# Zhaohuai-L/Any-Stereo

Hardware: AMD Instinct MI355X
Metric: stereo pairs/sec (coreContinuous_IGEV inference, 32-iter GRU, 960x540) (higher is better)
Workload: dtype f32 (3xf16 split-precision MFMA, fp32 accumulate); 1 GPU; coreContinuous_IGEV inference, 960x540 SceneFlow-shape synthetic pair (padded 960x544), 32 GRU iters, scale 1.0, Q=518400 queries, 1 pair(s) per GPU, random-init weights; pairs_per_gpu=1, parallelism=replicas x1, gru_loop=hipGraph

## Files before the change

any-stereo_amd/csrc/conv.hip:

```cpp
#include <stdlib.h>

#include <type_traits>

#include "common.h"
#include "conv_plan.h"
#include "split.h"

namespace {

using namespace as;

struct ConvParams {
  const float* src[AS_MAX_SRCS];
  int src_c[AS_MAX_SRCS];
  int src_end[AS_MAX_SRCS];
  int n_src;
  const float* wpack;
  const float* bias;
  const float* add;
  int add_ctot, add_coff;
  const float* h;
  const float* z;
  float* out;
  float* out2;
  int out_ctot, out_coff;
  int B, H, W, Cin, Cout, Cout_pad, act;
  int Hi, Wi;
  int tiles_x, tiles_y, n_tiles, chunks;
  int src_bs[AS_MAX_SRCS];
  _Float16* out_bs;
  int out_bs_c8tot, out_bs_coff8;
  int out_bs_ctot;
  int bs_only;
  int all_bs;
  int dual;
  const float* src2;
  int src2_bs;
  const float* wpack2;
  const float* bias2;
  int out_coff2, out_bs_coff8_2;
  const float* h2;
  int act2;
  int dual_sep;
  float* out_b;
  _Float16* out_bs_b;
  const float* tap_w;
  int xcd_map;
  int fast16;
  int ksplit;
  float* ws;
  int stagger;
  int lean_offset;
};

constexpr int kEpiTaps = AS_EPI_RELU_TAPS;

template <int KS> struct ConvCfg;
template <> struct ConvCfg<3> { static constexpr int KC = 8; };
template <> struct ConvCfg<1> { static constexpr int KC = 32; };
static_assert(ConvCfg<3>::KC == conv_kc(3) && ConvCfg<1>::KC == conv_kc(1), "conv_igemm_kernel's K chunk is the planner's");

struct EpiCtx {
  __amdgpu_buffer_rsrc_t r_add, r_out, r_h, r_z, r_bs, r_bsl;
  bool has_add, has_bs, skip_out;
  int act;
  int cvalid;
  int cend;
  unsigned plane4;
};

template <int EPI>
__device__ __forceinline__ EpiCtx make_epi_ctx(const ConvParams& p, int b, int n0, int bn, bool second = false) {
  EpiCtx e;
  const long long plane = (long long)p.H * p.W;
  const int cvalid = min(p.Cout - n0, bn);
  const int recs = cvalid > 0 ? (int)((long long)cvalid * plane * 4) : 0;
  e.plane4 = (unsigned)(plane * 4);
  e.act = second ? p.act2 : p.act;
  const bool sep = second && p.dual_sep;
  e.has_add = p.add != nullptr;
  const float* addp = p.add ? p.add + ((long long)b * p.add_ctot + p.add_coff + n0) * plane : p.out;
  e.r_add = __builtin_amdgcn_make_buffer_rsrc((void*)addp, 0, p.add ? recs : 0, 0x00020000);
  if (EPI == kEpiPartial) {
    const int ks = (int)(blockIdx.x / ((unsigned)p.B * p.tiles_x * p.tiles_y * p.n_tiles));
    float* dst = p.ws + (((long long)ks * p.B + b) * p.Cout_pad + n0) * plane;
    e.r_out = __builtin_amdgcn_make_buffer_rsrc((void*)dst, 0, (int)((long long)bn * plane * 4), 0x00020000);
    e.r_add = __builtin_amdgcn_make_buffer_rsrc((void*)dst, 0, 0, 0x00020000);
    e.has_add = false;
    e.r_h = e.r_out;
    e.r_z = e.r_out;
  } else if (EPI == AS_EPI_LINEAR) {
    float* outp = sep ? p.out_b + ((long long)b * p.Cout + n0) * plane
                      : p.out + ((long long)b * p.out_ctot + (second ? p.out_coff2 : p.out_coff) + n0) * plane;
    e.r_out = __builtin_amdgcn_make_buffer_rsrc((void*)outp, 0, recs, 0x00020000);
    const float* hsel = second ? p.h2 : p.h;
    const float* res = hsel ? hsel + ((long long)b * p.Cout + n0) * plane : outp;
    e.r_h = __builtin_amdgcn_make_buffer_rsrc((void*)res, 0, hsel ? recs : 0, 0x00020000);
    e.r_z = e.r_out;
  } else if (EPI == AS_EPI_GRU_ZR) {
    const int ch = p.Cout >> 1;
    const bool is_r = n0 >= ch;
    const int c0 = is_r ? n0 - ch : n0;
    float* dst = (is_r ? p.out2 : p.out) + ((long long)b * ch + c0) * plane;
    e.r_out = __builtin_amdgcn_make_buffer_rsrc((void*)dst, 0, recs, 0x00020000);
    e.r_h = __builtin_amdgcn_make_buffer_rsrc((void*)(p.h + ((long long)b * ch + c0) * plane), 0, is_r ? recs : 0, 0x00020000);
    e.r_z = e.r_out;
  } else {
    const long long o = ((long long)b * p.Cout + n0) * plane;
    e.r_out = __builtin_amdgcn_make_buffer_rsrc((void*)(p.out + o), 0, recs, 0x00020000);
    e.r_h = __builtin_amdgcn_make_buffer_rsrc((void*)(p.h + o), 0, recs, 0x00020000);
    e.r_z = __builtin_amdgcn_make_buffer_rsrc((void*)(p.z + o), 0, recs, 0x00020000);
  }
  e.has_bs = false;
  e.skip_out = false;
  e.cvalid = cvalid;
  e.cend = cvalid;
  e.r_bs = e.r_out;
  e.r_bsl = e.r_out;
  if (EPI != kEpiPartial && (sep ? p.out_bs_b != nullptr : p.out_bs != nullptr)) {
    int c0 = n0;
    bool on = true;
    if (EPI == AS_EPI_GRU_ZR) { const int ch = p.Cout >> 1; on = n0 >= ch; c0 = n0 - ch; }
    if (on) {
      const int nblk = cvalid > 0 ? (cvalid + 7) / 8 : 0;
      const int coff8 = sep ? 0 : (second ? p.out_bs_coff8_2 : p.out_bs_coff8);
      const int c8tot = sep ? (p.Cout + 7) / 8 : p.out_bs_c8tot;
      _Float16* dst = (sep ? p.out_bs_b : p.out_bs) + (((long long)b * 2 * c8tot + coff8 + (c0 >> 3)) * plane) * 8;
      e.r_bs = __builtin_amdgcn_make_buffer_rsrc((void*)dst, 0, (int)((long long)nblk * plane * 16), 0x00020000);
      e.r_bsl = __builtin_amdgcn_make_buffer_rsrc((void*)(dst + (long long)c8tot * plane * 8), 0, (int)((long long)nblk * plane * 16), 0x00020000);
      e.has_bs = true;
      e.cend = (sep ? p.Cout : p.out_bs_ctot) - (coff8 * 8 + c0);
      e.skip_out = p.bs_only != 0;
    }
  }
  return e;
}

__device__ unsigned g_split_overflow_conv;

struct EpiRegs {
  unsigned off[8];
  float av[8], hv[8], zv[8];
};

template <int EPI>
__device__ __forceinline__ void epi_load(const EpiCtx& e, int col0, int half, unsigned poff, int g, EpiRegs& R) {
  constexpr unsigned kOOB = 0x7FFFFFF0u;
#pragma unroll
  for (int i = 0; i < 8; ++i) {
    const int r = g * 8 + i;
    const int col = col0 + (r & 3) + 8 * (r >> 2) + 4 * half;
    R.off[i] = poff == kOOB ? kOOB : (unsigned)col * e.plane4 + poff;
    R.av[i] = bload(e.r_add, R.off[i]);
    if (EPI == AS_EPI_GRU_ZR || EPI == AS_EPI_LINEAR) R.hv[i] = bload(e.r_h, R.off[i]);
    if (EPI == AS_EPI_GRU_Q) { R.hv[i] = bload(e.r_h, R.off[i]); R.zv[i] = bload(e.r_z, R.off[i]); }
  }
}

// ... 245 lines not shown
#pragma unroll
  for (int t = 0; t < 4; ++t) {
    if (t == wave) continue;
    const int slot = t * 3 + (wave < t ? wave : wave - 1);
    float* dst = lds + slot * 1024 + lane;
#pragma unroll
    for (int r = 0; r < 16; ++r) dst[r * 64] = acc[t >> 1][t & 1][r];
  }
  __syncthreads();
  f32x16 sum;
  {
    const f32x16 own = (wave == 0) ? acc[0][0] : (wave == 1) ? acc[0][1] : (wave == 2) ? acc[1][0] : acc[1][1];
    sum = own;
    const float* srcp = lds + wave * 3 * 1024 + lane;
#pragma unroll
    for (int s = 0; s < 3; ++s)
#pragma unroll
      for (int r = 0; r < 16; ++r) sum[r] += srcp[s * 1024 + r * 64];
  }

  __syncthreads();
  if (tid < kBN) lds[tid] = (p.bias && n0 + tid < p.Cout) ? p.bias[n0 + tid] : 0.f;
  __syncthreads();
  {
    const EpiCtx e = make_epi_ctx<EPI>(p, b, n0, kBN);
    const int m = (wave & 1) * 32 + l31;
    const int gy = y0 + m / TW, gx = x0 + m % TW;
    const unsigned poff = (gy < p.H && gx < p.W) ? (unsigned)(((long long)gy * p.W + gx) * 4) : 0x7FFFFFF0u;
    const bool is_r = (EPI == AS_EPI_GRU_ZR) && n0 >= (p.Cout >> 1);
    epilogue_tile<EPI>(p, e, sum, (wave >> 1) * 32, half, poff, lds, is_r);
  }
}

__global__ void pack_weights_kernel(const float* __restrict__ w, float* __restrict__ wp, int Cin, int Cout,
                                    int Cout_pad, int KS, int KC, long long total) {
  const long long idx = (long long)blockIdx.x * 256 + threadIdx.x;
  if (idx >= total) return;
  const int co = (int)(idx % Cout_pad);
  long long t = idx / Cout_pad;
  const int cl = (int)(t % KC);
  t /= KC;
  const int tap = (int)(t % (KS * KS));
  const int chunk = (int)(t / (KS * KS));
  const int ci = chunk * KC + cl;
  float v = 0.f;
  if (co < Cout && ci < Cin) v = w[((long long)co * Cin + ci) * KS * KS + tap];
  wp[idx] = v;
}


__global__ __launch_bounds__(256) void conv7x7_c1_kernel(const float* __restrict__ x, const float* __restrict__ w,
                                                         const float* __restrict__ bias, float* __restrict__ out,
                                                         int H, int W, int Cout, int out_ctot, int out_coff) {
  __shared__ float patch[22 * 22];
  const int b = blockIdx.z;
  const int x0 = blockIdx.x * 16, y0 = blockIdx.y * 16;
  const long long plane = (long long)H * W;
  const float* xp = x + (long long)b * plane;
  for (int idx = threadIdx.x; idx < 22 * 22; idx += 256) {
    const int py = idx / 22, px = idx - py * 22;
    const int gy = y0 - 3 + py, gx = x0 - 3 + px;
    patch[idx] = (gy >= 0 && gy < H && gx >= 0 && gx < W) ? xp[(long long)gy * W + gx] : 0.f;
  }
  __syncthreads();
  const int ly = threadIdx.x >> 4, lx = threadIdx.x & 15;
  float win[49];
#pragma unroll
  for (int t = 0; t < 49; ++t) win[t] = patch[(ly + t / 7) * 22 + lx + t % 7];
  const int gy = y0 + ly, gx = x0 + lx;
  const bool ok = gy < H && gx < W;
  float* o = out + ((long long)b * out_ctot + out_coff) * plane + (long long)gy * W + gx;
  for (int co = 0; co < Cout; ++co) {
    float acc = 0.f;
#pragma unroll
    for (int t = 0; t < 49; ++t) acc += win[t] * w[co * 49 + t];
    acc += bias ? bias[co] : 0.f;
    if (ok) o[(long long)co * plane] = fmaxf(acc, 0.f);
  }
}

__device__ __forceinline__ void bs8_store(_Float16* __restrict__ out_bs, long long b, int c8tot, int blk, long long plane,
                                          long long pix, const float (&v)[8], float& amax) {
  half8 hi, lo;
  amax = amax8(v, amax);
  split_mode8(v, hi, lo);
  _Float16* rec = out_bs + ((b * 2 * c8tot + blk) * plane + pix) * 8;
  *reinterpret_cast<half8*>(rec) = hi;
  *reinterpret_cast<half8*>(rec + (long long)c8tot * plane * 8) = lo;
}

template <int CO>
__global__ __launch_bounds__(256) void conv7x7_c1_tm_kernel(const float* __restrict__ x, const float* __restrict__ wt,
                                                            const float* __restrict__ bias, float* __restrict__ out,
                                                            int H, int W, int Cout, int CP, int out_ctot, int out_coff,
                                                            float* __restrict__ copy_out, int copy_ctot, int copy_coff, int copy_bs,
                                                            int out_bs) {
  __shared__ float patch[22 * 22];
  as::fp16_saturate_mode();
  float ovf_amax = 0.f;
  const int groups = CP / CO;
  const int b = blockIdx.z / groups;
  const int c0 = (blockIdx.z - b * groups) * CO;
  const int x0 = blockIdx.x * 16, y0 = blockIdx.y * 16;
  const long long plane = (long long)H * W;
  const __amdgpu_buffer_rsrc_t rs = __builtin_amdgcn_make_buffer_rsrc((void*)(x + (long long)b * plane), 0, (int)(plane * 4), 0x00020000);
  for (int idx = threadIdx.x; idx < 22 * 22; idx += 256) {
    const int py = idx / 22, px = idx - py * 22;
    const int gy = y0 - 3 + py, gx = x0 - 3 + px;
    patch[idx] = bload(rs, (gy >= 0 && gy < H && gx >= 0 && gx < W) ? (unsigned)((gy * W + gx) * 4) : 0x7FFFFFF0u);
  }
  __syncthreads();
  const int ly = threadIdx.x >> 4, lx = threadIdx.x & 15;
  float acc[CO];
#pragma unroll
  for (int j = 0; j < CO; ++j) acc[j] = 0.f;
#pragma unroll 1
  for (int ky = 0; ky < 7; ++ky) {
    const float* pr = patch + (ly + ky) * 22 + lx;
    const float* wr = wt + (ky * 7) * CP + c0;
#pragma unroll
    for (int kx = 0; kx < 7; ++kx) {
      const float v = pr[kx];
#pragma unroll
      for (int j = 0; j < CO; ++j) acc[j] = fmaf(v, wr[kx * CP + j], acc[j]);
    }
  }
  const int gy = y0 + ly, gx = x0 + lx;
  if (gy < H && gx < W) {
    if (out_bs) {
      static_assert(CO == 8, "blocked output: one 8-channel block per thread");
      if (c0 < (Cout + 7) / 8 * 8) {
        float v[8];
#pragma unroll
        for (int j = 0; j < CO; ++j) v[j] = (c0 + j < Cout) ? fmaxf(acc[j] + (bias ? bias[c0 + j] : 0.f), 0.f) : 0.f;
        bs8_store(reinterpret_cast<_Float16*>(out), b, (out_ctot + 7) >> 3, (out_coff + c0) >> 3, plane, (long long)gy * W + gx, v, ovf_amax);
      }
    } else {
      float* o = out + ((long long)b * out_ctot + out_coff + c0) * plane + (long long)gy * W + gx;
#pragma unroll
      for (int j = 0; j < CO; ++j)
        if (c0 + j < Cout) o[(long long)j * plane] = fmaxf(acc[j] + (bias ? bias[c0 + j] : 0.f), 0.f);
    }
    if (copy_out && c0 == 0) {
      const float v = patch[(ly + 3) * 22 + lx + 3];
      if (copy_bs) {
        const int c8 = (copy_ctot + 7) >> 3;
        _Float16* rec = reinterpret_cast<_Float16*>(copy_out) + (((long long)b * 2 * c8 + (copy_coff >> 3)) * plane + (long long)gy * W + gx) * 8 + (copy_coff & 7);
        const _Float16 hk = split_hi(v);
        rec[0] = hk;
        rec[(long long)c8 * plane * 8] = split_lo(v, hk);
        ovf_amax = fmaxf(ovf_amax, fabsf(v));
      } else {
        copy_out[((long long)b * copy_ctot + copy_coff) * plane + (long long)gy * W + gx] = v;
      }
    }
  }
  as::note_split_overflow(ovf_amax, &g_split_overflow_conv);
}

__global__ __launch_bounds__(256) void conv3x3_to1_kernel(const float* __restrict__ x, const float* __restrict__ w,
                                                          const float* __restrict__ bias, float* __restrict__ out,
                                                          int Cin, int H, int W) {
  __shared__ float red[4][64];
  const int lx = threadIdx.x & 63, slice = threadIdx.x >> 6;
  const int gx = blockIdx.x * 64 + lx, gy = blockIdx.y, b = blockIdx.z;
  const long long plane = (long long)H * W;
  const int c0 = slice * ((Cin + 3) / 4), c1 = min(Cin, c0 + (Cin + 3) / 4);
  float acc = 0.f;
  if (gx < W) {
    for (int c = c0; c < c1; ++c) {
      const float* xp = x + ((long long)b * Cin + c) * plane;
      const float* wc = w + c * 9;
#pragma unroll
      for (int ky = 0; ky < 3; ++ky) {
        const int yy = gy + ky - 1;
        if (yy < 0 || yy >= H) continue;
#pragma unroll
        for (int kx = 0; kx < 3; ++kx) {
          const int xx = gx + kx - 1;
          const float v = (xx >= 0 && xx < W) ? xp[(long long)yy * W + xx] : 0.f;
          acc += v * wc[ky * 3 + kx];
        }
      }
    }
  }
  red[slice][lx] = acc;
  __syncthreads();
  if (slice == 0 && gx < W)
    out[(long long)b * plane + (long long)gy * W + gx] = ((red[0][lx] + red[1][lx]) + (red[2][lx] + red[3][lx])) + (bias ? bias[0] : 0.f);
}

__global__ __launch_bounds__(256) void tap_shift_sum_kernel(const float* __restrict__ S, const float* __restrict__ bias,
                                                            const float* __restrict__ addend, float* __restrict__ out, int H,
                                                            int W, long long P, int groups) {
  const long long pix = (long long)blockIdx.x * 256 + threadIdx.x;
  if (pix >= P) return;
  const long long plane = (long long)H * W;
  const long long b = pix / plane;
  const int rem = (int)(pix - b * plane);
  const int y = rem / W, x = rem - y * W;
  const float* sp = S + b * groups * 9 * plane;
  float acc = 0.f;
  const __amdgpu_buffer_rsrc_t rs = __builtin_amdgcn_make_buffer_rsrc((void*)sp, 0, (int)((long long)groups * 9 * plane * 4), 0x00020000);
  unsigned toff[9];
#pragma unroll
  for (int t = 0; t < 9; ++t) {
    const int yy = y + t / 3 - 1, xx = x + t % 3 - 1;
    toff[t] = (yy >= 0 && yy < H && xx >= 0 && xx < W) ? (unsigned)(((long long)t * plane + (long long)yy * W + xx) * 4) : 0x7FFFFFF0u;
  }
  const unsigned gstep = (unsigned)(9 * plane * 4);
  for (int g0 = 0; g0 < groups; g0 += 4) {
    float v[4][9];
#pragma unroll
    for (int g = 0; g < 4; ++g)
#pragma unroll
      for (int t = 0; t < 9; ++t)
        v[g][t] = bload(rs, (toff[t] == 0x7FFFFFF0u || g0 + g >= groups) ? 0x7FFFFFF0u : toff[t] + (unsigned)(g0 + g) * gstep);
#pragma unroll
    for (int g = 0; g < 4; ++g)
#pragma unroll
      for (int t = 0; t < 9; ++t) acc += v[g][t];
  }
  const float delta = acc + (bias ? bias[0] : 0.f);
  out[pix] = addend ? addend[pix] + delta : delta;
}

__device__ __forceinline__ float pool2x_at(const float* __restrict__ xp, int yo, int xo, int H, int W) {
  float s = 0.f;
#pragma unroll
  for (int dy = 0; dy < 3; ++dy) {
    const int yy = 2 * yo - 1 + dy;
    if (yy < 0 || yy >= H) continue;
#pragma unroll
    for (int dx = 0; dx < 3; ++dx) {
      const int xx = 2 * xo - 1 + dx;
      if (xx >= 0 && xx < W) s += xp[(long long)yy * W + xx];
    }
  }
  return s / 9.f;
}

__global__ __launch_bounds__(256) void pool2x_kernel(const float* __restrict__ x, float* __restrict__ out, int H, int W,
                                                     int Ho, int Wo, long long total) {
  const long long idx = (long long)blockIdx.x * 256 + threadIdx.x;
  if (idx >= total) return;
  const int xo = (int)(idx % Wo);
  long long t = idx / Wo;
  const int yo = (int)(t % Ho);
  const long long bc = t / Ho;
  out[idx] = pool2x_at(x + bc * H * W, yo, xo, H, W);
}

__global__ __launch_bounds__(256) void pool2x_bs_kernel(const float* __restrict__ x, _Float16* __restrict__ out_bs, int C, int H, int W,
                                                        int Ho, int Wo, long long total) {
  const long long idx = (long long)blockIdx.x * 256 + threadIdx.x;
  as::fp16_saturate_mode();
  float ovf_amax = 0.f;
  if (idx >= total) return;
  const int c8 = (C + 7) >> 3;
  const int xo = (int)(idx % Wo);
  long long t = idx / Wo;
  const int yo = (int)(t % Ho);
  t /= Ho;
  const int blk = (int)(t % c8);
  const long long b = t / c8;
  const long long plane = (long long)H * W;
  const int nch = min(8, C - blk * 8);
  const __amdgpu_buffer_rsrc_t rs = __builtin_amdgcn_make_buffer_rsrc((void*)(x + (b * C + blk * 8) * plane), 0, (int)(nch * plane * 4), 0x00020000);
  unsigned off[9];
#pragma unroll
  for (int k = 0; k < 9; ++k) {
    const int yy = 2 * yo - 1 + k / 3, xx = 2 * xo - 1 + k % 3;
    off[k] = (yy >= 0 && yy < H && xx >= 0 && xx < W) ? (unsigned)(((long long)yy * W + xx) * 4) : 0x7FFFFFF0u;
  }
  const unsigned pl4 = (unsigned)(plane * 4);
  float raw[8][9];
#pragma unroll
  for (int j = 0; j < 8; ++j)
#pragma unroll
    for (int k = 0; k < 9; ++k) raw[j][k] = bload(rs, off[k] == 0x7FFFFFF0u ? off[k] : off[k] + (unsigned)j * pl4);
  float v[8];
#pragma unroll
  for (int j = 0; j < 8; ++j) {
    float sacc = 0.f;
#pragma unroll
    for (int k = 0; k < 9; ++k) sacc += raw[j][k];
    v[j] = sacc / 9.f;
  }
  bs8_store(out_bs, b, c8, blk, (long long)Ho * Wo, (long long)yo * Wo + xo, v, ovf_amax);
  as::note_split_overflow(ovf_amax, &g_split_overflow_conv);
}

__global__ __launch_bounds__(256) void pool2x_bs_even_kernel(const float* __restrict__ x, _Float16* __restrict__ out_bs, int C, int H, int W,
                                                             int Ho, int Wo, long long total) {
  const long long idx0 = (long long)blockIdx.x * 256 + threadIdx.x;
  as::fp16_saturate_mode();
  float ovf_amax = 0.f;
  const bool live = idx0 < total;
  const long long idx = live ? idx0 : total - 1;
  const int c8 = (C + 7) >> 3;
  const int xo = (int)(idx % Wo);
  long long t = idx / Wo;
  const int yo = (int)(t % Ho);
  t /= Ho;
  const int blk = (int)(t % c8);
  const long long b = t / c8;
// ... 935 lines not shown
  static_assert(!LEAN || lds <= 80 * 1024, "conv_split (lean): two blocks per CU");
  static bool configured = false;
  if (!configured && lds > 64 * 1024) {
    (void)hipFuncSetAttribute((const void*)conv_split_kernel<KS, TW, BN, EPI, NSUB, S, FAST, LEAN>, hipFuncAttributeMaxDynamicSharedMemorySize, lds);
    configured = true;
  }
  hipLaunchKernelGGL((conv_split_kernel<KS, TW, BN, EPI, NSUB, S, FAST, LEAN>), dim3((unsigned)pl.grid), dim3(pl.block), pl.lds, s, p);
  return as::check_launch("conv2d(split)");
}

template <int... Vs> struct Among {};
template <class F> bool conv_switch(F f) { f(); return true; }
template <class F, int... Vs, class... Rest>
bool conv_switch(F f, Among<Vs...>, int v, Rest... rest) {
  return ((v == Vs && conv_switch([&](auto... cs) { f(std::integral_constant<int, Vs>{}, cs...); }, rest...)) || ...);
}

int conv_launch(const ConvParams& p, const ConvPlan& pl, hipStream_t s) {
  int rc = 1;
  if (pl.family == kConvIgemm) {
    conv_switch([&](auto ks, auto tw, auto epi) {
      if constexpr (conv_igemm_valid(ks(), tw(), epi())) {
        hipLaunchKernelGGL((conv_igemm_kernel<ks(), tw(), epi()>), dim3((unsigned)pl.grid), dim3(pl.block), 0, s, p);
        rc = as::check_launch("conv2d");
      }
    }, Among<1, 3>{}, pl.KS, Among<8, 16, 32, 64>{}, pl.TW, Among<0, 1, 2>{}, pl.epilogue);
  } else if (pl.family == kConvSplit) {
    conv_switch([&](auto ks, auto tw, auto bn, auto epi, auto nsub, auto st, auto fast, auto lean) {
      if constexpr (conv_split_valid(ks(), tw(), bn(), epi(), nsub(), st(), fast(), lean()))
        rc = launch_conv_split<ks(), tw(), bn(), epi(), nsub(), st(), fast() != 0, lean() != 0>(p, pl, s);
    }, Among<1, 3>{}, pl.KS, Among<16, 32, 128>{}, pl.TW, Among<64, 128>{}, pl.BN, Among<0, 1, 2, 3, 4>{}, pl.epilogue,
       Among<1, 2>{}, pl.NSUB, Among<1, 2>{}, pl.S, Among<0, 1>{}, pl.FAST != 0, Among<0, 1>{}, pl.LEAN != 0);
  }
  return rc <= 0 ? rc : conv_no_kernel(pl);
}

int conv_run(const as_conv_desc& d, const ConvPlan& pl, hipStream_t s) {
  const ConvParams p = conv_fill_params(d, pl);
  const int rc = conv_launch(p, pl, s);
  if (rc != AS_OK || !pl.finish) return rc;
  const dim3 g((unsigned)pl.finish_grid);
  if (pl.finish_epilogue == AS_EPI_LINEAR) hipLaunchKernelGGL(conv_finish_kernel<AS_EPI_LINEAR>, g, dim3(256), 0, s, p);
  else if (pl.finish_epilogue == AS_EPI_GRU_ZR) hipLaunchKernelGGL(conv_finish_kernel<AS_EPI_GRU_ZR>, g, dim3(256), 0, s, p);
  else hipLaunchKernelGGL(conv_finish_kernel<AS_EPI_GRU_Q>, g, dim3(256), 0, s, p);
  return as::check_launch("conv2d(split-K finish)");
}

}

bool as::conv_has_kernel(const as_conv_plan& pl) {
  return pl.family == kConvIgemm ? conv_igemm_valid(pl.KS, pl.TW, pl.epilogue)
                                 : pl.family == kConvSplit && conv_split_valid(pl.KS, pl.TW, pl.BN, pl.epilogue, pl.NSUB, pl.S, pl.FAST != 0, pl.LEAN != 0);
}

extern "C" {

#ifdef AS_CONV_STAMPS
int as_debug_conv_stamps(unsigned long long* out, int n) {
  if (!out || n <= 0 || n > kStampBlocks * kStampSlots) return AS_ERR_BAD_ARG;
  if (hipMemcpyFromSymbol(out, HIP_SYMBOL(as_conv_stamp_buf), sizeof(unsigned long long) * n) != hipSuccess) return AS_ERR_LAUNCH;
  static unsigned long long zeros[kStampBlocks * kStampSlots];
  if (hipMemcpyToSymbol(HIP_SYMBOL(as_conv_stamp_buf), zeros, sizeof(zeros)) != hipSuccess) return AS_ERR_LAUNCH;
  return AS_OK;
}
int as_debug_conv_life(unsigned long long* out, int n) {
  if (!out || n <= 0 || n > kStampBlocks * 8) return AS_ERR_BAD_ARG;
  if (hipMemcpyFromSymbol(out, HIP_SYMBOL(as_conv_life_buf), sizeof(unsigned long long) * n) != hipSuccess) return AS_ERR_LAUNCH;
  return AS_OK;
}
#endif

int64_t as_conv_pack_size(int Cin, int Cout, int KS) {
  if (Cin <= 0 || Cout <= 0 || (KS != 1 && KS != 3)) return -1;
  const int KC = conv_kc(KS);
  const int64_t chunks = (Cin + KC - 1) / KC;
  return chunks * KS * KS * KC * conv_cout_pad(Cout);
}

int as_conv_pack_weights(const float* weight, float* wpack, int Cin, int Cout, int KS, void* stream) {
  AS_REQUIRE(weight && wpack, AS_ERR_BAD_ARG, "conv_pack: null pointer");
  const int64_t total = as_conv_pack_size(Cin, Cout, KS);
  AS_REQUIRE(total > 0, AS_ERR_BAD_ARG, "conv_pack: unsupported Cin=%d Cout=%d KS=%d", Cin, Cout, KS);
  hipLaunchKernelGGL(pack_weights_kernel, dim3((unsigned)as::cdiv64(total, 256)), dim3(256), 0, as::as_stream(stream),
                     weight, wpack, Cin, Cout, conv_cout_pad(Cout), KS, conv_kc(KS), (long long)total);
  return as::check_launch("conv_pack_weights");
}

int64_t as_conv_pack_size_split(int Cin, int Cout, int KS) {
  if (Cin <= 0 || Cout <= 0 || (KS != 1 && KS != 3)) return -1;
  int64_t chunks = (Cin + kSplitKC - 1) / kSplitKC;
  if (KS == 1) chunks = (chunks + 3) / 4 * 4;
  return chunks * KS * KS * 4 * conv_cout_pad(Cout) * 8;
}

int as_conv_pack_weights_split_t(const float* weight, void* wpack, int Cin, int Cout, int KS, void* stream) {
  AS_REQUIRE(weight && wpack, AS_ERR_BAD_ARG, "conv_pack_split_t: null pointer");
  const int64_t total = as_conv_pack_size_split(Cin, Cout, KS);
  AS_REQUIRE(total > 0, AS_ERR_BAD_ARG, "conv_pack_split_t: unsupported Cin=%d Cout=%d KS=%d", Cin, Cout, KS);
  hipLaunchKernelGGL(pack_weights_split_kernel, dim3((unsigned)as::cdiv64(total, 256)), dim3(256), 0, as::as_stream(stream),
                     weight, (_Float16*)wpack, Cin, Cout, conv_cout_pad(Cout), KS * KS, (long long)total, 1);
  return as::check_launch("conv_pack_weights_split_t");
}

int as_conv_pack_weights_split(const float* weight, void* wpack, int Cin, int Cout, int KS, void* stream) {
  AS_REQUIRE(weight && wpack, AS_ERR_BAD_ARG, "conv_pack_split: null pointer");
  const int64_t total = as_conv_pack_size_split(Cin, Cout, KS);
  AS_REQUIRE(total > 0, AS_ERR_BAD_ARG, "conv_pack_split: unsupported Cin=%d Cout=%d KS=%d", Cin, Cout, KS);
  hipLaunchKernelGGL(pack_weights_split_kernel, dim3((unsigned)as::cdiv64(total, 256)), dim3(256), 0, as::as_stream(stream),
                     weight, (_Float16*)wpack, Cin, Cout, conv_cout_pad(Cout), KS * KS, (long long)total, 0);
  return as::check_launch("conv_pack_weights_split");
}

int64_t as_conv_ws_elems(int B, int Cout, int H, int W) {
  if (B <= 0 || Cout <= 0 || H <= 0 || W <= 0) return 0;
  const int cpad = conv_cout_pad(Cout);
  const int bn = (cpad % 128 == 0) ? 128 : 64;
  const long long tiles = (long long)B * as::cdiv64((long long)H * W, 128) * (cpad / bn);
  const int ks = conv_ksplit_cap(tiles, 8);
  return ks > 1 ? (int64_t)ks * B * cpad * H * W : 0;
}

int as_conv2d(const as_conv_desc* d, void* stream) {
  int rc = as::conv_validate(d);
  if (rc != AS_OK) return rc;
  const int fast16 = as::fast16_mode();
  hipStream_t s = as::as_stream(stream);
  ConvPlan pl;
  if ((rc = conv_plan(*d, conv_knobs(), fast16, &pl)) != AS_OK) return rc;
  if (pl.dual != kDualSequential) return conv_run(*d, pl, s);
  as_conv_desc first = *d;
  first.dual = 0;
  const as_conv_desc second = as::conv_dual_second(*d);
  ConvPlan pl2;
  if ((rc = as::conv_validate(&second)) != AS_OK || (rc = conv_plan(second, conv_knobs(), fast16, &pl2)) != AS_OK) return rc;
  if ((rc = conv_run(first, pl, s)) != AS_OK) return rc;
  return conv_run(second, pl2, s);
}

int as_conv7x7_c1_relu(const float* x, const float* weight, const float* bias, float* out, int B, int H, int W,
                       int Cout, int out_ctot, int out_coff, int tap_major, float* copy_out, int copy_ctot, int copy_coff,
                       int copy_bs, int out_bs, void* stream) {
  AS_REQUIRE(x && weight && out, AS_ERR_BAD_ARG, "conv7x7_c1: null pointer");
  AS_REQUIRE((long long)H * W * 4 < 0x7FFFFFF0ll, AS_ERR_BAD_SHAPE, "conv7x7_c1: plane too large");
  AS_REQUIRE(B > 0 && H > 0 && W > 0 && Cout > 0, AS_ERR_BAD_ARG, "conv7x7_c1: non-positive size");
  AS_REQUIRE(out_coff >= 0 && out_coff + Cout <= (out_bs ? (out_ctot + 7) / 8 * 8 : out_ctot), AS_ERR_BAD_SHAPE, "conv7x7_c1: out channel window outside out_ctot");
  AS_REQUIRE(!out_bs || (out_coff % 8 == 0 && (reinterpret_cast<uintptr_t>(out) & 15) == 0), AS_ERR_BAD_ARG, "conv7x7_c1: blocked output window must start at a multiple of 8, 16-B aligned");
  AS_REQUIRE(B <= 65535 && as::cdiv(H, 16) <= 65535, AS_ERR_BAD_SHAPE, "conv7x7_c1: grid too large");
  dim3 grid((unsigned)as::cdiv(W, 16), (unsigned)as::cdiv(H, 16), (unsigned)B);
  if (tap_major) {
    const int CP = (Cout + 63) / 64 * 64;
    AS_REQUIRE((long long)B * (CP / 8) <= 65535, AS_ERR_BAD_SHAPE, "conv7x7_c1: grid too large");
    const dim3 g3(grid.x, grid.y, (unsigned)(B * (CP / 8)));
    AS_REQUIRE(!copy_out || (copy_coff >= 0 && copy_coff < copy_ctot), AS_ERR_BAD_SHAPE, "conv7x7_c1: copy channel outside copy_ctot");
    hipLaunchKernelGGL(conv7x7_c1_tm_kernel<8>, g3, dim3(256), 0, as::as_stream(stream), x, weight, bias, out, H, W, Cout, CP, out_ctot, out_coff,
                       copy_out, copy_ctot, copy_coff, copy_bs, out_bs);
  } else {
    AS_REQUIRE(!out_bs, AS_ERR_BAD_ARG, "conv7x7_c1: a blocked output needs tap_major weights");
    AS_REQUIRE(!copy_out, AS_ERR_BAD_ARG, "conv7x7_c1: the input pass-through needs tap_major weights");
    hipLaunchKernelGGL(conv7x7_c1_kernel, grid, dim3(256), 0, as::as_stream(stream), x, weight, bias, out, H, W, Cout, out_ctot, out_coff);
  }
  return as::check_launch("conv7x7_c1_relu");
}

int as_conv3x3_to1(const float* x, const float* weight, const float* bias, float* out, int B, int Cin, int H, int W, void* stream) {
  AS_REQUIRE(x && weight && out, AS_ERR_BAD_ARG, "conv3x3_to1: null pointer");
  AS_REQUIRE(B > 0 && H > 0 && W > 0 && Cin > 0, AS_ERR_BAD_ARG, "conv3x3_to1: non-positive size");
  AS_REQUIRE(B <= 65535 && H <= 65535, AS_ERR_BAD_SHAPE, "conv3x3_to1: grid too large");
  dim3 grid((unsigned)as::cdiv(W, 64), (unsigned)H, (unsigned)B);
  hipLaunchKernelGGL(conv3x3_to1_kernel, grid, dim3(256), 0, as::as_stream(stream), x, weight, bias, out, Cin, H, W);
  return as::check_launch("conv3x3_to1");
}

int as_tap_shift_sum(const float* S, const float* bias, const float* addend, float* out, int B, int H, int W, int groups, void* stream) {
  AS_REQUIRE(S && out, AS_ERR_BAD_ARG, "tap_shift_sum: null pointer");
  AS_REQUIRE(B > 0 && H > 0 && W > 0 && groups > 0, AS_ERR_BAD_ARG, "tap_shift_sum: non-positive size");
  const long long P = (long long)B * H * W;
  hipLaunchKernelGGL(tap_shift_sum_kernel, dim3((unsigned)as::cdiv64(P, 256)), dim3(256), 0, as::as_stream(stream), S, bias, addend, out, H, W, P, groups);
  return as::check_launch("tap_shift_sum");
}

int as_pool2x(const float* x, float* out, int B, int C, int H, int W, void* stream) {
  AS_REQUIRE(x && out, AS_ERR_BAD_ARG, "pool2x: null pointer");
  AS_REQUIRE(B > 0 && C > 0 && H > 0 && W > 0, AS_ERR_BAD_ARG, "pool2x: non-positive size");
  const int Ho = (H - 1) / 2 + 1, Wo = (W - 1) / 2 + 1;
  const long long total = (long long)B * C * Ho * Wo;
  hipLaunchKernelGGL(pool2x_kernel, dim3((unsigned)as::cdiv64(total, 256)), dim3(256), 0, as::as_stream(stream), x, out, H, W, Ho, Wo, total);
  return as::check_launch("pool2x");
}

int as_interp_bilinear_ac(const float* x, float* out, int B, int C, int H, int W, int Ho, int Wo, void* stream) {
  AS_REQUIRE(x && out, AS_ERR_BAD_ARG, "interp: null pointer");
  AS_REQUIRE(B > 0 && C > 0 && H > 0 && W > 0 && Ho > 0 && Wo > 0, AS_ERR_BAD_ARG, "interp: non-positive size");
  const float sy = Ho > 1 ? (float)(H - 1) / (float)(Ho - 1) : 0.f;
  const float sx = Wo > 1 ? (float)(W - 1) / (float)(Wo - 1) : 0.f;
  const long long total = (long long)B * C * Ho * Wo;
  hipLaunchKernelGGL(interp_kernel, dim3((unsigned)as::cdiv64(total, 256)), dim3(256), 0, as::as_stream(stream), x, out, H, W, Ho, Wo, sy, sx, total);
  return as::check_launch("interp_bilinear_ac");
}

int as_pool2x_bs(const float* x, void* out_bs, int B, int C, int H, int W, void* stream) {
  AS_REQUIRE(x && out_bs, AS_ERR_BAD_ARG, "pool2x_bs: null pointer");
  AS_REQUIRE(B > 0 && C > 0 && H > 0 && W > 0, AS_ERR_BAD_ARG, "pool2x_bs: non-positive size");
  AS_REQUIRE((reinterpret_cast<uintptr_t>(out_bs) & 15) == 0, AS_ERR_BAD_ARG, "pool2x_bs: out_bs not 16-B aligned");
  const int Ho = (H - 1) / 2 + 1, Wo = (W - 1) / 2 + 1;
  const long long total = (long long)B * ((C + 7) / 8) * Ho * Wo;
  static const int even_mode = getenv("AS_POOL2X_EVEN") ? atoi(getenv("AS_POOL2X_EVEN")) : 1;
  if (even_mode && (W & 1) == 0 && (reinterpret_cast<uintptr_t>(x) & 7) == 0 && (long long)H * W * 4 * 8 < 0x7FFFFFF0ll)
    hipLaunchKernelGGL(pool2x_bs_even_kernel, dim3((unsigned)as::cdiv64(total, 256)), dim3(256), 0, as::as_stream(stream), x,
                       reinterpret_cast<_Float16*>(out_bs), C, H, W, Ho, Wo, total);
  else
    hipLaunchKernelGGL(pool2x_bs_kernel, dim3((unsigned)as::cdiv64(total, 256)), dim3(256), 0, as::as_stream(stream), x,
                       reinterpret_cast<_Float16*>(out_bs), C, H, W, Ho, Wo, total);
  return as::check_launch("pool2x_bs");
}

int as_interp_bilinear_ac_bs(const float* x, void* out_bs, int B, int C, int H, int W, int Ho, int Wo, void* stream) {
  AS_REQUIRE(x && out_bs, AS_ERR_BAD_ARG, "interp_bs: null pointer");
  AS_REQUIRE(B > 0 && C > 0 && H > 0 && W > 0 && Ho > 0 && Wo > 0, AS_ERR_BAD_ARG, "interp_bs: non-positive size");
  AS_REQUIRE((reinterpret_cast<uintptr_t>(out_bs) & 15) == 0, AS_ERR_BAD_ARG, "interp_bs: out_bs not 16-B aligned");
  const float sy = Ho > 1 ? (float)(H - 1) / (float)(Ho - 1) : 0.f;
  const float sx = Wo > 1 ? (float)(W - 1) / (float)(Wo - 1) : 0.f;
  const long long total = (long long)B * ((C + 7) / 8) * Ho * Wo;
  hipLaunchKernelGGL(interp_bs_kernel, dim3((unsigned)as::cdiv64(total, 256)), dim3(256), 0, as::as_stream(stream), x,
                     reinterpret_cast<_Float16*>(out_bs), C, H, W, Ho, Wo, sy, sx, total);
  return as::check_launch("interp_bilinear_ac_bs");
}

unsigned as_conv_split_overflow(int reset) { return as::read_reset_counter(&g_split_overflow_conv, reset); }

}
```

Measured before the change: 52.49 pairs/s.

## Run the single-channel 7x7 conv on fp32 MFMA tiles

Adds an MFMA-based kernel for the 7x7 conv with one input channel. It treats the 49 taps as a K dimension in 25 steps of the fp32 32x32x2 instruction, with a shared-memory input patch and a lane shuffle to rearrange outputs before the stores. It is selected by default when Cout is a multiple of 32, with an environment variable to turn it off. This targets the scalar FMA cost of the older tap-major kernel, at the price of more register pressure and extra shuffle work.

Measured after the change: 52.74 pairs/s, median of 3. No clear change (+0.5%).

```diff
diff --git a/any-stereo_amd/csrc/conv.hip b/any-stereo_amd/csrc/conv.hip
--- a/any-stereo_amd/csrc/conv.hip
+++ b/any-stereo_amd/csrc/conv.hip
@@ -4,6 +4,7 @@
 
 #include "common.h"
 #include "conv_plan.h"
+#include "mfma_f32.h"
 #include "split.h"
 
 namespace {
@@ -555,6 +556,112 @@
         ovf_amax = fmaxf(ovf_amax, fabsf(v));
       } else {
         copy_out[((long long)b * copy_ctot + copy_coff) * plane + (long long)gy * W + gx] = v;
+      }
+    }
+  }
+  as::note_split_overflow(ovf_amax, &g_split_overflow_conv);
+}
+
+__device__ __forceinline__ void conv7x7_c1_store8(const float (&a)[8], int cb, int b, long long plane, long long pix, bool inside,
+                                                  const float* bias8, float* __restrict__ out, int Cout, int out_ctot,
+                                                  int out_coff, int out_bs, float& ovf_amax) {
+  if (!inside || cb >= Cout) return;
+  float v[8];
+#pragma unroll
+  for (int j = 0; j < 8; ++j) v[j] = fmaxf(a[j] + bias8[j], 0.f);
+  if (out_bs) {
+    bs8_store(reinterpret_cast<_Float16*>(out), b, (out_ctot + 7) >> 3, (out_coff + cb) >> 3, plane, pix, v, ovf_amax);
+  } else {
+    float* o = out + ((long long)b * out_ctot + out_coff + cb) * plane + pix;
+#pragma unroll
+    for (int j = 0; j < 8; ++j) o[(long long)j * plane] = v[j];
+  }
+}
+
+template <int TH, int NCT>
+__global__ __launch_bounds__(256) void conv7x7_c1_mfma_kernel(const float* __restrict__ x, const float* __restrict__ wt,
+                                                              const float* __restrict__ bias, float* __restrict__ out,
+                                                              int H, int W, int Cout, int CP, int out_ctot, int out_coff,
+                                                              float* __restrict__ copy_out, int copy_ctot, int copy_coff, int copy_bs,
+                                                              int out_bs) {
+  static_assert(TH % 2 == 0, "a pixel tile of the MFMA is two rows of 16");
+  constexpr int PW = 22, PH = TH + 6;
+  __shared__ float patch[PH * PW];
+  __shared__ __attribute__((aligned(16))) float bias_s[32 * NCT];
+  as::fp16_saturate_mode();
+  float ovf_amax = 0.f;
+  const int groups = CP / (32 * NCT);
+  const int b = blockIdx.z / groups;
+  const int c0 = (blockIdx.z - b * groups) * (32 * NCT);
+  const int x0 = blockIdx.x * 16, y0 = blockIdx.y * TH;
+  const long long plane = (long long)H * W;
+  const int lane = threadIdx.x & 63;
+  const int wave = __builtin_amdgcn_readfirstlane(threadIdx.x >> 6);
+  const int h = as::mfma32_k(lane), n = as::mfma32_rc(lane);
+  float wa[NCT][25];
+#pragma unroll
+  for (int s = 0; s < 25; ++s) {
+    const bool real = (s < 24) || h == 0;
+    const float* wr = wt + (real ? 2 * s + h : 0) * CP + c0 + n;
+#pragma unroll
+    for (int ct = 0; ct < NCT; ++ct) wa[ct][s] = real ? wr[32 * ct] : 0.f;
+  }
+  const __amdgpu_buffer_rsrc_t rs = __builtin_amdgcn_make_buffer_rsrc((void*)(x + (long long)b * plane), 0, (int)(plane * 4), 0x00020000);
+  for (int idx = threadIdx.x; idx < PH * PW; idx += 256) {
+    const int py = idx / PW, px = idx - py * PW;
+    const int gy = y0 - 3 + py, gx = x0 - 3 + px;
+    patch[idx] = bload(rs, (gy >= 0 && gy < H && gx >= 0 && gx < W) ? (unsigned)((gy * W + gx) * 4) : 0x7FFFFFF0u);
+  }
+  if (threadIdx.x < 32 * NCT) bias_s[threadIdx.x] = (bias && c0 + (int)threadIdx.x < Cout) ? bias[c0 + threadIdx.x] : 0.f;
+  __syncthreads();
+  for (int pt = wave; pt < TH / 2; pt += 4) {
+    const int py = 2 * pt + (n >> 4), px = n & 15;
+    const float* p0 = patch + py * PW + px;
+    const float* p1 = p0 + h;
+    const float* p16 = p0 + 16 * h;
+    f32x16 acc[NCT] = {};
+#pragma unroll
+    for (int s = 0; s < 25; ++s) {
+      const int t = 2 * s, off = (t / 7) * PW + t % 7;
+      float bv;
+      if (s == 24) {
+        bv = p0[off];
+        bv = h ? 0.f : bv;
+      } else {
+        bv = (t % 7 == 6) ? p16[off] : p1[off];
+      }
+#pragma unroll
+      for (int ct = 0; ct < NCT; ++ct) acc[ct] = as::chain_step(wa[ct][s], bv, acc[ct]);
+    }
+    const int gy = y0 + py, gx = x0 + px;
+    const bool inside = gy < H && gx < W;
+    const long long pix = (long long)gy * W + gx;
+#pragma unroll
+    for (int ct = 0; ct < NCT; ++ct) {
+#pragma unroll
+      for (int q = 0; q < 2; ++q) {
+        float v[8];
+#pragma unroll
+        for (int j = 0; j < 4; ++j) {
+          const float xq = acc[ct][4 * q + j], yq = acc[ct][4 * (q + 2) + j];
+          const float recv = __shfl_xor(h ? xq : yq, 32);
+          v[j] = h ? recv : xq;
+          v[4 + j] = h ? yq : recv;
+        }
+        conv7x7_c1_store8(v, c0 + 32 * ct + 8 * (q + 2 * h), b, plane, pix, inside, bias_s + 32 * ct + 8 * (q + 2 * h), out, Cout, out_ctot, out_coff, out_bs, ovf_amax);
+      }
+    }
+    if (copy_out && c0 == 0 && h == 0 && inside) {
+      const float v = patch[(py + 3) * PW + px + 3];
+      if (copy_bs) {
+        const int c8 = (copy_ctot + 7) >> 3;
+        _Float16* rec = reinterpret_cast<_Float16*>(copy_out) + (((long long)b * 2 * c8 + (copy_coff >> 3)) * plane + pix) * 8 + (copy_coff & 7);
+        const _Float16 hk = split_hi(v);
+        rec[0] = hk;
+        rec[(long long)c8 * plane * 8] = split_lo(v, hk);
+        ovf_amax = fmaxf(ovf_amax, fabsf(v));
+      } else {
+        copy_out[((long long)b * copy_ctot + copy_coff) * plane + pix] = v;
       }
     }
   }
@@ -1796,6 +1903,15 @@
     AS_REQUIRE((long long)B * (CP / 8) <= 65535, AS_ERR_BAD_SHAPE, "conv7x7_c1: grid too large");
     const dim3 g3(grid.x, grid.y, (unsigned)(B * (CP / 8)));
     AS_REQUIRE(!copy_out || (copy_coff >= 0 && copy_coff < copy_ctot), AS_ERR_BAD_SHAPE, "conv7x7_c1: copy channel outside copy_ctot");
+    static const int mfma = getenv("AS_CONV7X7_MFMA") ? atoi(getenv("AS_CONV7X7_MFMA")) : 1;
+    if (mfma && Cout % 32 == 0) {
+      AS_REQUIRE(as::cdiv(H, 8) <= 65535, AS_ERR_BAD_SHAPE, "conv7x7_c1: grid too large");
+      AS_REQUIRE((long long)B * (CP / 32) <= 65535, AS_ERR_BAD_SHAPE, "conv7x7_c1: grid too large");
+      hipLaunchKernelGGL((conv7x7_c1_mfma_kernel<8, 1>), dim3(grid.x, (unsigned)as::cdiv(H, 8), (unsigned)(B * (CP / 32))), dim3(256), 0,
+                         as::as_stream(stream), x, weight, bias, out, H, W, Cout, CP, out_ctot, out_coff, copy_out, copy_ctot, copy_coff,
+                         copy_bs, out_bs);
+      return as::check_launch("conv7x7_c1_relu");
+    }
     hipLaunchKernelGGL(conv7x7_c1_tm_kernel<8>, g3, dim3(256), 0, as::as_stream(stream), x, weight, bias, out, H, W, Cout, CP, out_ctot, out_coff,
                        copy_out, copy_ctot, copy_coff, copy_bs, out_bs);
   } else {
diff --git a/any-stereo_amd/csrc/mfma_f32.h b/any-stereo_amd/csrc/mfma_f32.h
--- /dev/null
+++ b/any-stereo_amd/csrc/mfma_f32.h
@@ -0,0 +1,19 @@
+#pragma once
+#include "split.h"
+
+namespace as {
+
+constexpr int kMfma32K = 2;
+constexpr int kMfma16K = 4;
+
+__device__ __forceinline__ int mfma32_k(int lane) { return lane >> 5; }
+__device__ __forceinline__ int mfma32_rc(int lane) { return lane & 31; }
+__device__ __forceinline__ int mfma32_row(int lane, int r) { return (r & 3) + 8 * (r >> 2) + 4 * (lane >> 5); }
+__device__ __forceinline__ int mfma16_k(int lane) { return lane >> 4; }
+__device__ __forceinline__ int mfma16_rc(int lane) { return lane & 15; }
+__device__ __forceinline__ int mfma16_row(int lane, int r) { return 4 * (lane >> 4) + r; }
+
+__device__ __forceinline__ f32x16 chain_step(float a, float b, f32x16 acc) { return __builtin_amdgcn_mfma_f32_32x32x2f32(a, b, acc, 0, 0, 0); }
+__device__ __forceinline__ f32x4 chain_step(float a, float b, f32x4 acc) { return __builtin_amdgcn_mfma_f32_16x16x4f32(a, b, acc, 0, 0, 0); }
+
+}
```
